# vmware/splinterdb

Hardware: AMD Instinct MI355X
Metric: routing_filter build Mkeys/s + probe Mkeys/s, device-resident, 24B keys (higher is better)
Workload: dtype u32; 1 GPU; C2: 64M x 24B keys per GPU = 8 filters x 8,000,000, build + full probe; filters_total=8, filters_per_gpu=8, keys_per_filter=8000000, key_len=24, fingerprint_size=26, log_index_size=8, seed=42, parallelism=key-range shards, 1 rank(s), no data-path collective

## Files before the change

### splinterdb_amd/csrc/rf_kernels.hip

```cpp
#include <hip/hip_runtime.h>
#include <stdint.h>

#include <atomic>

#include "rf_device.h"
#include "rf_plan.h"
#include "rf_launch.h"

using namespace rf;

typedef unsigned int v4u __attribute__((ext_vector_type(4)));
typedef unsigned int v2u __attribute__((ext_vector_type(2)));

template <int KIND, bool NT = false>
__device__ __forceinline__ uint32_t hash_key(const void* __restrict__ in0, const uint64_t* __restrict__ offs,
                                             uint32_t key_len, uint32_t seed, uint64_t k) {
  if constexpr (KIND == IN_KEYS24) {
    const v2u* kp = reinterpret_cast<const v2u*>(static_cast<const uint8_t*>(in0) + k * 24);
    v2u a, b, c;
    if constexpr (NT) {
      a = __builtin_nontemporal_load(kp);
      b = __builtin_nontemporal_load(kp + 1);
      c = __builtin_nontemporal_load(kp + 2);
    } else {
      a = kp[0];
      b = kp[1];
      c = kp[2];
    }
    uint32_t w[6] = {a.x, a.y, b.x, b.y, c.x, c.y};
    return xxh32_24(w, seed);
  } else if constexpr (KIND == IN_KEYS_W) {
    return xxh32_words(reinterpret_cast<const uint32_t*>(static_cast<const uint8_t*>(in0) + k * key_len),
                       key_len, seed);
  } else if constexpr (KIND == IN_KEYS_B) {
    const uint8_t* kp = static_cast<const uint8_t*>(in0) + k * key_len;
    return NT ? xxh32_unaligned_prefetch(kp, key_len, seed) : xxh32_unaligned(kp, key_len, seed);
  } else if constexpr (KIND == IN_VAR) {
    const uint64_t o0 = offs[k], o1 = offs[k + 1];
    const uint8_t* kp = static_cast<const uint8_t*>(in0) + o0;
    return NT ? xxh32_unaligned_prefetch(kp, (uint32_t)(o1 - o0), seed) : xxh32_unaligned(kp, (uint32_t)(o1 - o0), seed);
  } else {
    if constexpr (NT) return __builtin_nontemporal_load(static_cast<const uint32_t*>(in0) + k);
    else return static_cast<const uint32_t*>(in0)[k];
  }
}

#define KEY_KIND_CASES(L)              \
  case IN_KEYS24: L(IN_KEYS24); break; \
  case IN_KEYS_W: L(IN_KEYS_W); break; \
  case IN_KEYS_B: L(IN_KEYS_B); break; \
  case IN_VAR: L(IN_VAR); break;
#define KIND_SWITCH(kind, L)    \
  switch (kind) {               \
    KEY_KIND_CASES(L)           \
    default: L(IN_HASH); break; \
  }

__device__ __forceinline__ uint32_t select64_fast(uint64_t x, uint32_t r) {
  uint32_t pos = 0;
#pragma unroll
  for (uint32_t w = 32; w >= 1; w >>= 1) {
    const uint32_t c = __popcll(x & ((1ull << w) - 1));
    if (r >= c) { r -= c; x >>= w; pos += w; }
  }
  return pos;
}
__device__ __forceinline__ uint64_t lowmask64(uint32_t k) { return k >= 64 ? ~0ull : ((1ull << k) - 1); }

__device__ __forceinline__ uint32_t xcd_chunk(uint32_t b, uint32_t nb) {
  const uint32_t q = nb / 8, r = nb % 8, xcd = b % 8;
  return (xcd < r ? xcd * (q + 1) : r * (q + 1) + (xcd - r) * q) + b / 8;
}

__device__ __forceinline__ void cb_scan_filter(const FilterPlan& P, const uint32_t* counts, uint32_t* cb_count,
                                               uint32_t* cb_start, uint32_t* cb_cursor, uint32_t* s_tmp,
                                               bool fresh) {
  const uint32_t num_cb = 1u << P.cbits;
  constexpr uint32_t PER = MAX_CB / 256;
  uint32_t v[PER], sum = 0;
#pragma unroll
  for (uint32_t k = 0; k < PER; k++) {
    const uint32_t i = threadIdx.x * PER + k;
    v[k] = 0;
    if (i < num_cb)
      v[k] = fresh ? __hip_atomic_load(&counts[P.cb_base + i], __ATOMIC_RELAXED, __HIP_MEMORY_SCOPE_AGENT)
                   : counts[P.cb_base + i];
    sum += v[k];
  }
  uint32_t total;
  uint32_t run = block_excl_scan<256>(sum, s_tmp, &total);
#pragma unroll
  for (uint32_t k = 0; k < PER; k++) {
    const uint32_t i = threadIdx.x * PER + k;
    if (i < num_cb) {
      cb_count[P.cb_base + i] = v[k];
      cb_start[P.cb_base + i] = run;
      cb_cursor[P.cb_base + i] = run;
    }
    run += v[k];
  }
}

struct TileRuns {
  const uint32_t* value;
  const uint32_t* end;
};

struct CountFold {
  uint32_t* outs_words;
  uint32_t num_out_words;
  uint32_t* ticket;
  uint32_t* cb_count;
  uint32_t* cb_start;
  uint32_t num_filters;
};

template <int KIND, typename EntT, bool FL = (sizeof(EntT) == 8), bool RUNS = false>
__global__ __launch_bounds__(TILE_NT) void k_hash_count(const FilterPlan* __restrict__ plans,
                                                        const uint32_t* __restrict__ tile_filter,
                                                        const uint32_t* __restrict__ tile_start,
                                                        const void* __restrict__ in0,
                                                        const uint64_t* __restrict__ offs,
                                                        uint32_t key_len, uint32_t fp_size,
                                                        uint32_t seed, EntT* __restrict__ ent,
                                                        uint32_t* cb_count,
                                                        const uint32_t* __restrict__ gate, uint32_t num_tiles,
                                                        CountFold fold, TileRuns runs) {
  __shared__ uint32_t s_hist[MAX_CB];
  if (fold.outs_words && blockIdx.x == 0)
    for (uint32_t i = threadIdx.x; i < fold.num_out_words; i += TILE_NT) fold.outs_words[i] = 0;
  if (gate && *gate == 0) return;
  for (uint32_t t = blockIdx.x; t < num_tiles; t += gridDim.x) {
  const FilterPlan& P = plans[tile_filter[t]];
  const uint32_t start = tile_start[t];
  const uint32_t count = RUNS ? runs.end[t] - start : min((uint32_t)TILE_KEYS, P.num_new - start);
  const uint32_t value = RUNS ? runs.value[t] : P.value;
  const uint32_t num_cb = 1u << P.cbits;
  __syncthreads();
  for (uint32_t i = threadIdx.x; i < num_cb; i += TILE_NT) s_hist[i] = 0;
  __syncthreads();
  const uint32_t esh = fp_size + P.vs - P.cbits;
  for (uint32_t j = threadIdx.x; j < count; j += TILE_NT) {
    const uint32_t h = hash_key<KIND>(in0, offs, key_len, seed, P.key_first + start + j);
    const uint32_t e = ((h >> (32 - fp_size)) << P.vs) | value;
    if constexpr (FL) {
      ent[P.e_first + start + j] = (EntT)(((EntT)e << 1) | EntT(1));
    } else {
      ent[P.e_first + start + j] = e;
    }
    const uint32_t cb = P.cbits ? (e >> esh) : 0u;
    atomicAdd(&s_hist[cb], 1u);
  }
  __syncthreads();
  for (uint32_t i = threadIdx.x; i < num_cb; i += TILE_NT) {
    const uint32_t c = s_hist[i];
    if (c) atomicAdd(&cb_count[P.cb_base + i], c);
  }
  }
  if (fold.ticket) {
    static_assert(TILE_NT == 256, "cb_scan_filter's workgroup");
    __shared__ uint32_t s_last;
    __threadfence();
    __syncthreads();
    if (threadIdx.x == 0) s_last = atomicAdd(fold.ticket, 1u) == gridDim.x - 1 ? 1u : 0u;
    __syncthreads();
    if (!s_last) return;
    __threadfence();
    if (threadIdx.x == 0) *fold.ticket = 0;
    for (uint32_t f = 0; f < fold.num_filters; f++)
      cb_scan_filter(plans[f], cb_count, fold.cb_count, fold.cb_start, cb_count, s_hist, true);
  }
}

__global__ __launch_bounds__(TILE_NT) void k_old_count(const FilterPlan* __restrict__ plans,
                                                       const uint32_t* __restrict__ tile_filter,
                                                       const uint32_t* __restrict__ tile_start,
                                                       uint32_t fp_size,
                                                       const uint64_t* __restrict__ ent,
                                                       uint32_t* __restrict__ cb_count) {
  __shared__ uint32_t s_hist[MAX_CB];
  const uint32_t t = blockIdx.x;
  const FilterPlan& P = plans[tile_filter[t]];
  const uint32_t start = tile_start[t];
  const uint32_t count = min((uint32_t)TILE_KEYS, P.old_region - start);
  const uint32_t num_cb = 1u << P.cbits;
  for (uint32_t i = threadIdx.x; i < num_cb; i += TILE_NT) s_hist[i] = 0;
  __syncthreads();
  const uint32_t esh = fp_size + P.vs - P.cbits;
  for (uint32_t j = threadIdx.x; j < count; j += TILE_NT) {
    const uint64_t x = ent[P.e_first + P.num_new + start + j];
    if (x == ~0ull) continue;
    const uint32_t e = (uint32_t)(x >> 1);
    atomicAdd(&s_hist[P.cbits ? (e >> esh) : 0u], 1u);
  }
  __syncthreads();
  for (uint32_t i = threadIdx.x; i < num_cb; i += TILE_NT) {
    const uint32_t c = s_hist[i];
    if (c) atomicAdd(&cb_count[P.cb_base + i], c);
  }
}

__global__ __launch_bounds__(256) void k_cb_scan(const FilterPlan* __restrict__ plans,
                                                 const uint32_t* counts,
                                                 uint32_t* cb_count,
                                                 uint32_t* __restrict__ cb_start,
                                                 uint32_t* cb_cursor,
                                                 const uint32_t* __restrict__ gate) {
  __shared__ uint32_t s_tmp[256 / WAVE + 1];
  if (gate && *gate == 0) return;
  cb_scan_filter(plans[blockIdx.x], counts, cb_count, cb_start, cb_cursor, s_tmp, false);
}

template <typename EntT, bool FL = (sizeof(EntT) == 8), bool RUNS = false>
__global__ __launch_bounds__(SCAT_NT) void k_scatter(const FilterPlan* __restrict__ plans,
                                                     const uint32_t* __restrict__ tile_filter,
                                                     const uint32_t* __restrict__ tile_start,
                                                     uint32_t region_is_old, uint32_t fp_size,
                                                     const EntT* __restrict__ ent,
                                                     EntT* __restrict__ part,
                                                     uint32_t* __restrict__ cb_cursor,
                                                     const uint32_t* __restrict__ gate, uint32_t num_tiles,
                                                     TileRuns runs) {
  __shared__ EntT s_stage[TILE_KEYS];
  __shared__ uint32_t s_off[MAX_CB];
  __shared__ uint32_t s_tmp[SCAT_NT / WAVE + 1];
  if (gate && *gate == 0) return;
  constexpr int PER = TILE_KEYS / SCAT_NT;
  constexpr int BPT = MAX_CB / SCAT_NT;
  for (uint32_t t = blockIdx.x; t < num_tiles; t += gridDim.x) {
  __syncthreads();
  const FilterPlan& P = plans[tile_filter[t]];
  const uint32_t start = tile_start[t];
  const uint32_t region = region_is_old ? P.old_region : P.num_new;
  const uint64_t base = P.e_first + (region_is_old ? P.num_new : 0u) + start;
  const uint32_t count = (RUNS && !region_is_old) ? runs.end[t] - start : min((uint32_t)TILE_KEYS, region - start);
  const uint32_t num_cb = 1u << P.cbits;
  for (uint32_t i = threadIdx.x; i < num_cb; i += SCAT_NT) s_off[i] = 0;
  __syncthreads();
  const uint32_t esh = fp_size + P.vs - P.cbits;
  auto cb_of = [&](EntT x) -> uint32_t {
    uint32_t e;
    if constexpr (FL) e = (uint32_t)(x >> 1);
    else e = x;
    return P.cbits ? (e >> esh) : 0u;
  };
  EntT v[PER];
  uint32_t cbv[PER], rank[PER];
#pragma unroll
  for (int k = 0; k < PER; k++) v[k] = ent[base + min(threadIdx.x + k * SCAT_NT, count - 1)];
#pragma unroll
  for (int k = 0; k < PER; k++) {
    const uint32_t j = threadIdx.x + k * SCAT_NT;
    cbv[k] = ~0u;
    if (j < count) {
      bool valid = true;
      if constexpr (sizeof(EntT) == 8) valid = v[k] != ~0ull;
      if (valid) {
        cbv[k] = cb_of(v[k]);
        rank[k] = atomicAdd(&s_off[cbv[k]], 1u);
      }
    }
  }
  __syncthreads();
  uint32_t cnt[BPT], sum = 0;
#pragma unroll
  for (int k = 0; k < BPT; k++) {
    const uint32_t b = threadIdx.x * BPT + k;
    cnt[k] = b < num_cb ? s_off[b] : 0u;
    sum += cnt[k];
  }
  uint32_t valid_total;
  uint32_t run = block_excl_scan<SCAT_NT>(sum, s_tmp, &valid_total);
  uint32_t gbase[BPT];
#pragma unroll
  for (int k = 0; k < BPT; k++) {
    const uint32_t b = threadIdx.x * BPT + k;
    gbase[k] = 0;
    if (b < num_cb) {
      s_off[b] = run;
      if (cnt[k]) gbase[k] = atomicAdd(&cb_cursor[P.cb_base + b], cnt[k]) - run;
      run += cnt[k];
    }
  }
  __syncthreads();
#pragma unroll
  for (int k = 0; k < PER; k++) {
    if (cbv[k] != ~0u) s_stage[s_off[cbv[k]] + rank[k]] = v[k];
  }
  __syncthreads();
#pragma unroll
  for (int k = 0; k < BPT; k++) {
    const uint32_t b = threadIdx.x * BPT + k;
    if (b < num_cb) s_off[b] = gbase[k];
  }
  __syncthreads();
  EntT* dst = part + P.e_first;
  for (uint32_t j = threadIdx.x; j < valid_total; j += SCAT_NT) {
    const EntT x = s_stage[j];
    dst[s_off[cb_of(x)] + j] = x;
  }
  }
}

__device__ uint64_t* g_dbg_ts = nullptr;
__device__ uint32_t g_dbg_kid = 0;
#ifdef RF_PHASE_STAMPS
#define DBG_PHASE_K(kid, k)                                                  \
  do {                                                                       \
    uint64_t* _ts = g_dbg_ts;                                                \
    if (_ts && g_dbg_kid == (kid) && threadIdx.x == 0)                       \
      _ts[blockIdx.x * 16 + (k)] = __builtin_amdgcn_s_memtime();             \
  } while (0)
#else
#define DBG_PHASE_K(kid, k) \
  do {                      \
  } while (0)
#endif
#define DBG_PHASE(k) DBG_PHASE_K(1, k)

extern "C" int rf_debug_set_phase_buffer(uint64_t* d_buf, uint32_t kid) {
  if (hipMemcpyToSymbol(HIP_SYMBOL(g_dbg_kid), &kid, sizeof(kid)) != hipSuccess) return 1;
  return hipMemcpyToSymbol(HIP_SYMBOL(g_dbg_ts), &d_buf, sizeof(d_buf)) == hipSuccess ? 0 : 1;
}

#ifndef RF_SCAT_WPE
#define RF_SCAT_WPE 4
#endif
template <int KIND, bool FL = false, bool RUNS = false, bool P16 = false>
__global__ __launch_bounds__(SCAT_NT) __attribute__((amdgpu_waves_per_eu(RF_SCAT_WPE))) void k_hash_scatter(const FilterPlan* __restrict__ plans,
                                                          const uint32_t* __restrict__ tile_filter,
                                                          const uint32_t* __restrict__ tile_start,
                                                          const void* __restrict__ in0,
                                                          const uint64_t* __restrict__ offs,
                                                          uint32_t key_len, uint32_t fp_size, uint32_t seed,
                                                          uint32_t* __restrict__ part,
                                                          uint32_t* __restrict__ cb_fill,
                                                          uint32_t* __restrict__ spill, TileRuns runs) {
  __shared__ __attribute__((aligned(16))) uint32_t s_stage[TILE_KEYS];
  __shared__ uint32_t s_off[MAX_CB];
  __shared__ uint32_t s_tmp[SCAT_NT / WAVE + 1];
  constexpr int PER = TILE_KEYS / SCAT_NT;
  constexpr int BPT = MAX_CB / SCAT_NT;
  static_assert(!P16 || (!FL && !RUNS), "16-bit keys: fresh single-run builds only");
  DBG_PHASE_K(2, 15);
  const uint32_t t = xcd_chunk(blockIdx.x, gridDim.x);
  const FilterPlan& P = plans[tile_filter[t]];
  const uint32_t start = tile_start[t];
  const uint32_t count = RUNS ? runs.end[t] - start : min((uint32_t)TILE_KEYS, P.num_new - start);
  const uint32_t value = RUNS ? runs.value[t] : P.value;
  const uint32_t num_cb = 1u << P.cbits;
  for (uint32_t i = threadIdx.x; i < num_cb; i += SCAT_NT) s_off[i] = 0;
  __syncthreads();
  DBG_PHASE_K(2, 0);
  const uint32_t esh = fp_size + P.vs - P.cbits + (FL ? 1u : 0u);
  auto cb_of = [&](uint32_t e) -> uint32_t { return P.cbits ? (e >> esh) : 0u; };
  const uint32_t flag = FL ? 1u : 0u;
  uint32_t v[PER], rank[PER];
  constexpr int HASH_CHUNK = 8;
  uint32_t dep = 0;
  constexpr bool X3 = KIND == IN_KEYS24;
  const uint32_t lane = threadIdx.x & (WAVE - 1);
  auto key_of = [&](int k) -> uint32_t {
    if constexpr (KIND == IN_VAR) return (threadIdx.x & ~(WAVE - 1)) * PER + k * WAVE + lane;
    else if constexpr (X3) return (threadIdx.x & ~(WAVE - 1)) + k * SCAT_NT + (lane >> 1) + (lane & 1) * 32;
    else return threadIdx.x + k * SCAT_NT;
  };
  constexpr uint32_t VWIN = (TILE_KEYS / (SCAT_NT / WAVE)) * 4 - 16;
  uint32_t* s_vwin = s_stage + (threadIdx.x / WAVE) * (TILE_KEYS / (SCAT_NT / WAVE));
  uint64_t vw0 = 0, vw1 = 0, vo0 = 0, vo1 = 0;
  if constexpr (KIND == IN_VAR) {
    const uint32_t j = min(key_of(0), count - 1);
    vo0 = offs[P.key_first + start + j];
    vo1 = offs[P.key_first + start + j + 1];
  }
#pragma unroll
  for (int k0 = 0; k0 < PER; k0 += HASH_CHUNK) {
    if constexpr (X3) {
      const uint32_t half = lane & 1, ki = lane >> 1;
      const uint8_t* kbase = static_cast<const uint8_t*>(in0) + (uint64_t)(P.key_first + start) * 24 + 12 * half;
      uint32_t a[HASH_CHUNK][3], b[HASH_CHUNK][3];
#pragma unroll
      for (int k = 0; k < HASH_CHUNK; k++) {
        const uint32_t c0 = (threadIdx.x & ~(WAVE - 1)) + (k0 + k) * SCAT_NT;
        const uint32_t ja = min(c0 + ki, count - 1) + dep, jb = min(c0 + 32 + ki, count - 1) + dep;
        const uint32_t* pa = reinterpret_cast<const uint32_t*>(kbase + (uint64_t)ja * 24);
        const uint32_t* pb = reinterpret_cast<const uint32_t*>(kbase + (uint64_t)jb * 24);
        a[k][0] = pa[0]; a[k][1] = pa[1]; a[k][2] = pa[2];
        b[k][0] = pb[0]; b[k][1] = pb[1]; b[k][2] = pb[2];
      }
#pragma unroll
      for (int k = 0; k < HASH_CHUNK; k++) {
        uint32_t w[6];
#pragma unroll
        for (int q = 0; q < 3; q++) {
          const uint32_t send = half ? a[k][q] : b[k][q];
          const uint32_t recv = (uint32_t)__builtin_amdgcn_mov_dpp((int)send, 0xB1, 0xf, 0xf, false);
          w[q] = half ? recv : a[k][q];
          w[3 + q] = half ? b[k][q] : recv;
        }
        const uint32_t h = xxh32_24(w, seed);
        v[k0 + k] = ((((h >> (32 - fp_size)) << P.vs) | value) << flag) | flag;
      }
    } else if constexpr (KIND == IN_KEYS24) {
      v2u ka[HASH_CHUNK], kb[HASH_CHUNK], kc[HASH_CHUNK];
#pragma unroll
      for (int k = 0; k < HASH_CHUNK; k++) {
        const uint32_t j = min(threadIdx.x + (k0 + k) * SCAT_NT, count - 1) + dep;
        const v2u* kp = reinterpret_cast<const v2u*>(static_cast<const uint8_t*>(in0) +
                                                     (uint64_t)(P.key_first + start + j) * 24);
        ka[k] = kp[0];
        kb[k] = kp[1];
        kc[k] = kp[2];
      }
      uint32_t z;
      asm volatile("v_mov_b32 %0, 0" : "=v"(z)
                   : "v"(ka[0].x), "v"(ka[1].x), "v"(ka[2].x), "v"(ka[3].x), "v"(ka[4].x), "v"(ka[5].x),
                     "v"(ka[6].x), "v"(ka[7].x), "v"(kb[0].x), "v"(kb[1].x), "v"(kb[2].x), "v"(kb[3].x),
                     "v"(kb[4].x), "v"(kb[5].x), "v"(kb[6].x), "v"(kb[7].x), "v"(kc[0].x), "v"(kc[1].x),
                     "v"(kc[2].x), "v"(kc[3].x), "v"(kc[4].x), "v"(kc[5].x), "v"(kc[6].x), "v"(kc[7].x));
#pragma unroll
      for (int k = 0; k < HASH_CHUNK; k++) {
        uint32_t w[6] = {ka[k].x + z, ka[k].y, kb[k].x, kb[k].y, kc[k].x, kc[k].y};
        const uint32_t h = xxh32_24(w, seed);
        v[k0 + k] = ((((h >> (32 - fp_size)) << P.vs) | value) << flag) | flag;
      }
    } else if constexpr (KIND == IN_VAR) {
#pragma unroll
      for (int k = 0; k < HASH_CHUNK; k++) {
        const uint64_t o0 = vo0, o1 = vo1;
        if (k0 + k + 1 < PER) {
          const uint32_t j = min(key_of(k0 + k + 1), count - 1);
          vo0 = offs[P.key_first + start + j];
          vo1 = offs[P.key_first + start + j + 1];
        }
        const uint32_t h = wave_hash_var<VWIN, false>(static_cast<const uint8_t*>(in0), o0, o1,
                                                      key_of(k0 + k) < count, s_vwin, seed, &vw0, &vw1);
        v[k0 + k] = ((((h >> (32 - fp_size)) << P.vs) | value) << flag) | flag;
      }
    } else {
#pragma unroll
      for (int k = k0; k < k0 + HASH_CHUNK; k++) {
        const uint32_t j = min(threadIdx.x + k * SCAT_NT, count - 1) + dep;
        const uint32_t h = hash_key<KIND>(in0, offs, key_len, seed, P.key_first + start + j);
        v[k] = ((((h >> (32 - fp_size)) << P.vs) | value) << flag) | flag;
      }
    }
    static_assert(HASH_CHUNK == 8, "opaque dependency below takes 8 hashes");
    asm volatile("v_mov_b32 %0, 0" : "=v"(dep)
                 : "v"(v[k0]), "v"(v[k0 + 1]), "v"(v[k0 + 2]), "v"(v[k0 + 3]), "v"(v[k0 + 4]),
                   "v"(v[k0 + 5]), "v"(v[k0 + 6]), "v"(v[k0 + 7]));
  }
  DBG_PHASE_K(2, 5);
#pragma unroll
  for (int k = 0; k < PER; k++) {
    if (key_of(k) < count) rank[k] = atomicAdd(&s_off[cb_of(v[k])], 1u);
  }
  __syncthreads();
  DBG_PHASE_K(2, 1);
  uint32_t cnt[BPT], sum = 0;
#pragma unroll
  for (int k = 0; k < BPT; k++) {
    const uint32_t b = threadIdx.x * BPT + k;
    cnt[k] = b < num_cb ? s_off[b] : 0u;
    sum += cnt[k];
  }
  uint32_t total;
  uint32_t run = block_excl_scan<SCAT_NT>(sum, s_tmp, &total);
  uint32_t g[BPT], lstart[BPT];
#pragma unroll
  for (int k = 0; k < BPT; k++) {
    const uint32_t b = threadIdx.x * BPT + k;
    g[k] = 0;
    lstart[k] = run;
    if (b < num_cb) {
      if (cnt[k]) g[k] = atomicAdd(&cb_fill[P.cb_base + b], cnt[k]);
      s_off[b] = run;
      run += cnt[k];
    }
  }
  __syncthreads();
  DBG_PHASE_K(2, 2);
#pragma unroll
  for (int k = 0; k < PER; k++) {
    if (key_of(k) < count) s_stage[s_off[cb_of(v[k])] + rank[k]] = v[k];
  }
  __syncthreads();
  DBG_PHASE_K(2, 3);
  bool over = false;
#pragma unroll
  for (int k = 0; k < BPT; k++) {
    const uint32_t b = threadIdx.x * BPT + k;
    if (b < num_cb) {
      over |= cnt[k] && g[k] + cnt[k] > (uint32_t)SORT_CAP;
      s_off[b] = g[k] - lstart[k];
    }
  }
  if (over) atomicOr(spill, 1u);
  __syncthreads();
  DBG_PHASE_K(2, 4);
  uint32_t* dst = part + P.e_first;
  if constexpr (P16) {
    auto reg16 = [&](uint32_t cb) -> uint16_t* { return reinterpret_cast<uint16_t*>(dst + (uint64_t)cb * CB_REGION); };
    for (uint32_t j = threadIdx.x; j < total; j += SCAT_NT) {
      const uint32_t x = s_stage[j];
      const uint32_t cb = cb_of(x);
      const uint32_t slot = s_off[cb] + j;
      if (slot < (uint32_t)SORT_CAP) reg16(cb)[slot] = (uint16_t)x;
    }
  } else {
    for (uint32_t j = threadIdx.x; j < total; j += SCAT_NT) {
      const uint32_t x = s_stage[j];
      const uint32_t cb = cb_of(x);
      const uint32_t slot = s_off[cb] + j;
      if (slot < (uint32_t)SORT_CAP) dst[(uint64_t)cb * CB_REGION + slot] = x;
    }
  }
  DBG_PHASE_K(2, 8);
}

template <typename EntT, bool FL = (sizeof(EntT) == 8)>
__device__ __forceinline__ uint32_t ent_e(EntT x) {
  if constexpr (FL) return (uint32_t)(x >> 1);
  else return x;
}
template <typename EntT, bool FL = (sizeof(EntT) == 8)>
__device__ __forceinline__ bool ent_drop(EntT x, EntT prev) {
  if constexpr (FL) return x == prev && (x & EntT(1));
  else return x == prev;
}

template <typename T>
__device__ __forceinline__ void sort8(T (&x)[8]) {
#define CE(a, b) { const T lo = x[a] < x[b] ? x[a] : x[b], hi = x[a] < x[b] ? x[b] : x[a]; x[a] = lo; x[b] = hi; }
  CE(0, 1) CE(2, 3) CE(4, 5) CE(6, 7) CE(0, 2) CE(1, 3) CE(4, 6) CE(5, 7) CE(1, 2) CE(5, 6)
  CE(0, 4) CE(1, 5) CE(2, 6) CE(3, 7) CE(2, 4) CE(3, 5) CE(1, 2) CE(3, 4) CE(5, 6)
#undef CE
}
template <typename T>
__device__ __forceinline__ void sort16(T (&x)[16]) {
#define CE(a, b) { const T lo = x[a] < x[b] ? x[a] : x[b], hi = x[a] < x[b] ? x[b] : x[a]; x[a] = lo; x[b] = hi; }
  CE(0, 1) CE(2, 3) CE(0, 2) CE(1, 3) CE(1, 2) CE(4, 5) CE(6, 7) CE(4, 6) CE(5, 7) CE(5, 6) CE(0, 4)
  CE(2, 6) CE(2, 4) CE(1, 5) CE(3, 7) CE(3, 5) CE(1, 2) CE(3, 4) CE(5, 6) CE(8, 9) CE(10, 11) CE(8, 10)
  CE(9, 11) CE(9, 10) CE(12, 13) CE(14, 15) CE(12, 14) CE(13, 15) CE(13, 14) CE(8, 12) CE(10, 14)
  CE(10, 12) CE(9, 13) CE(11, 15) CE(11, 13) CE(9, 10) CE(11, 12) CE(13, 14) CE(0, 8) CE(4, 12)
  CE(4, 8) CE(2, 10) CE(6, 14) CE(6, 10) CE(2, 4) CE(6, 8) CE(10, 12) CE(1, 9) CE(5, 13) CE(5, 9)
  CE(3, 11) CE(7, 15) CE(7, 11) CE(3, 5) CE(7, 9) CE(11, 13) CE(1, 2) CE(3, 4) CE(5, 6) CE(7, 8)
  CE(9, 10) CE(11, 12) CE(13, 14)
#undef CE
}

template <typename T, int NT>
__device__ void oe_sort_group(T* a, uint32_t cnt) {
  uint32_t n = 1;
  while (n < cnt) n <<= 1;
  for (uint32_t p = 1; p < n; p <<= 1) {
    for (uint32_t k = p; k >= 1; k >>= 1) {
      const uint32_t r = k & (p - 1);
      for (uint32_t L = threadIdx.x; L + k < cnt; L += NT) {
        if (L >= r && ((L - r) & (2 * k - 1)) < k && (L / (2 * p)) == ((L + k) / (2 * p))) {
          const T x = a[L], y = a[L + k];
          if (y < x) {
            a[L] = y;
            a[L + k] = x;
          }
        }
      }
      __syncthreads();
    }
  }
}

struct CbCtx {
  uint32_t rvs, vs, lis, bbits, idx0;
  uint32_t cb_rel;
  uint64_t e_first;
};

__device__ __forceinline__ void write_index_bounds(const CbCtx& c, const uint32_t* sorted, uint32_t kept,
                                                   uint32_t* idx_cnt, uint32_t* idx_start,
                                                   uint32_t* uniq_out) {
  const uint32_t ipc = 1u << (c.bbits - c.lis);
  const uint32_t ish = c.lis + c.rvs;
  for (uint32_t li = threadIdx.x; li < ipc; li += blockDim.x) {
    auto lb = [&](uint32_t key) {
      uint32_t lo = 0, hi = kept;
      while (lo < hi) {
        uint32_t mid = (lo + hi) >> 1;
        uint32_t m = ish >= 32 ? 0u : ((sorted[mid] >> ish) & (ipc - 1));
        if (m < key) lo = mid + 1; else hi = mid;
      }
      return lo;
    };
    const uint32_t lo = lb(li);
    const uint32_t hi = (li + 1 < ipc) ? lb(li + 1) : kept;
    idx_cnt[c.idx0 + li] = hi - lo;
    idx_start[c.idx0 + li] = c.cb_rel + lo;
  }
  uint32_t uniq = 0;
  for (uint32_t i = threadIdx.x; i < kept; i += blockDim.x) {
    const uint32_t fp = sorted[i] >> c.vs;
    const bool first = (i == 0) || (ish < 32 && ((sorted[i] >> ish) != (sorted[i - 1] >> ish)));
    const uint32_t prev = first ? (0xffffffffu >> c.vs) : (sorted[i - 1] >> c.vs);
    uniq += (fp != prev) ? 1u : 0u;
  }
  *uniq_out = uniq;
}

template <typename EntT, bool FL = (sizeof(EntT) == 8), bool DUAL = false, bool LIST = false, bool RUNS = false>
__global__ __launch_bounds__(SORT_NT, 6) void k_cb_sort(const FilterPlan* __restrict__ plans,
                                                     const uint32_t* __restrict__ cb_filter,
                                                     const uint32_t* __restrict__ cb_count,
                                                     const uint32_t* __restrict__ cb_start,
                                                     const EntT* __restrict__ part,
                                                     const uint32_t* __restrict__ old32,
                                                     const uint32_t* __restrict__ ob_lo,
                                                     const uint32_t* __restrict__ ob_n,
                                                     uint32_t* __restrict__ sorted32,
                                                     uint32_t* __restrict__ idx_cnt,
                                                     uint32_t* __restrict__ idx_start,
                                                     FilterOut* __restrict__ outs,
                                                     uint32_t* __restrict__ overflow,
                                                     uint32_t lis, uint32_t* __restrict__ first_old,
                                                     uint32_t* __restrict__ has_old,
                                                     const uint32_t* __restrict__ spill,
                                                     const uint32_t* __restrict__ cb_outs,
                                                     const uint32_t* __restrict__ cb_list) {
  constexpr int PER = SORT_CAP / SORT_NT;
  DBG_PHASE(15);
  __shared__ EntT s_b[SORT_CAP];
  __shared__ __attribute__((aligned(16))) uint32_t s_bin[MAX_BINS + 1];
  __shared__ uint32_t s_tmp[SORT_NT / WAVE + 1];
  static_assert(MAX_BINS + 1 >= 2048 + 2 * MAX_IPC && MAX_IPC + 1 <= 2048, "s_fo / s_ho inside s_bin");
  constexpr uint32_t BIG_LIST = 64;
  __shared__ uint32_t s_big[BIG_LIST];
  __shared__ uint32_t s_nbig;
  uint32_t* s_first = s_bin;
  uint32_t* s_fo = s_bin + 2048;
  uint32_t* s_ho = s_bin + 2048 + MAX_IPC;
  const uint32_t nit = LIST ? cb_list[0] : 1u;
  for (uint32_t it = LIST ? blockIdx.x : 0u; it < nit; it += LIST ? gridDim.x : 1u) {
  uint32_t cb;
  if constexpr (LIST) {
    cb = cb_list[1 + it];
    if (!(cb >> 31)) continue;
    cb &= 0x7fffffffu;
  } else {
    cb = xcd_chunk(blockIdx.x, gridDim.x);
  }
  const uint32_t f = cb_filter[cb];
  const FilterPlan& P = plans[f];
  const uint32_t n = cb_count[cb];
  const uint32_t cbl = cb - P.cb_base;
  const uint32_t cb_rel = (spill && *spill == 0) ? cbl * CB_REGION : cb_start[cb];
  const uint32_t cb_out = (DUAL && spill) ? cb_outs[cb] : cb_rel;
  CbCtx c{P.rvs, P.vs, lis, P.bbits, P.idx_base + (cbl << (P.bbits - lis)), cb_out, P.e_first};
  if (n > SORT_CAP) {
    if (threadIdx.x == 0 && !LIST) overflow[1 + atomicAdd(&overflow[0], 1u)] = cb;
    continue;
  }
  const uint32_t nbins = 1u << (P.bbits - P.binsh);
  const uint32_t bmask = nbins - 1, bsh = P.rvs + P.binsh;
  const uint32_t ipc = 1u << (P.bbits - lis), ish = lis + P.rvs;
  EntT v[PER];
  static_assert(SORT_CAP <= 65536 && PER % 2 == 0, "16-bit ranks, packed in pairs");
  uint32_t rp[PER / 2];
#pragma unroll
  for (int k = 0; k < PER / 2; k++) rp[k] = 0;
  const EntT* src = part + P.e_first + cb_rel;
  const uint32_t nm1 = n ? n - 1 : 0u;
  if constexpr (DUAL) {
    const uint32_t nn = n - ob_n[cb];
    const uint32_t* osrc = (P.old_direct ? P.old_entries : old32 + P.old_first) + ob_lo[cb];
#pragma unroll
    for (int k = 0; k < PER; k++) {
      const uint32_t j = min(threadIdx.x + k * SORT_NT, nm1);
      v[k] = *(j < nn ? reinterpret_cast<const uint32_t*>(src) + j : osrc + (j - nn));
    }
  } else {
#pragma unroll
    for (int k = 0; k < PER; k++) v[k] = src[min(threadIdx.x + k * SORT_NT, nm1)];
  }
  for (uint32_t i = threadIdx.x; i <= nbins; i += SORT_NT) s_bin[i] = 0;
  if (threadIdx.x == 0) s_nbig = 0;
  __builtin_amdgcn_fence(__ATOMIC_RELEASE, "workgroup", "local");
  __builtin_amdgcn_s_barrier();
  __builtin_amdgcn_fence(__ATOMIC_ACQUIRE, "workgroup", "local");
  DBG_PHASE(0);
  uint32_t nsort = n;
  if constexpr (DUAL) nsort = n - ob_n[cb];
#pragma unroll
  for (int k = 0; k < PER; k++) {
    if (threadIdx.x + k * SORT_NT < nsort) {
      const uint32_t e = ent_e<EntT, FL>(v[k]);
      const uint32_t b = bsh >= 32 ? 0u : ((e >> bsh) & bmask);
      rp[k / 2] |= atomicAdd(&s_bin[b], 1u) << (16 * (k & 1));
    }
  }
  __syncthreads();
  DBG_PHASE(1);
  {
    constexpr int BPT = MAX_BINS / SORT_NT;
    static_assert(BPT == 8, "two 16-byte accesses per thread");
    v4u* sb4 = reinterpret_cast<v4u*>(s_bin) + 2 * threadIdx.x;
    const bool own = threadIdx.x * BPT < nbins;
    v4u a = own ? sb4[0] : v4u{0u, 0u, 0u, 0u}, b = own ? sb4[1] : v4u{0u, 0u, 0u, 0u};
    if (own && nbins < BPT) {
      uint32_t t8[8] = {a.x, a.y, a.z, a.w, b.x, b.y, b.z, b.w};
#pragma unroll
      for (int k = 0; k < 8; k++) if ((uint32_t)k >= nbins) t8[k] = 0;
      a = v4u{t8[0], t8[1], t8[2], t8[3]};
      b = v4u{t8[4], t8[5], t8[6], t8[7]};
    }
    const uint32_t sum = a.x + a.y + a.z + a.w + b.x + b.y + b.z + b.w;
    uint32_t total;
    uint32_t run = block_excl_scan<SORT_NT>(sum, s_tmp, &total);
    v4u ea, eb;
    ea.x = run; run += a.x; ea.y = run; run += a.y; ea.z = run; run += a.z; ea.w = run; run += a.w;
    eb.x = run; run += b.x; eb.y = run; run += b.y; eb.z = run; run += b.z; eb.w = run;
    if (own && nbins >= BPT) {
      sb4[0] = ea;
      sb4[1] = eb;
    } else if (own) {
      const uint32_t e8[8] = {ea.x, ea.y, ea.z, ea.w, eb.x, eb.y, eb.z, eb.w};
      for (uint32_t k = 0; k < nbins; k++) s_bin[k] = e8[k];
    }
    if (threadIdx.x == 0) s_bin[nbins] = nsort;
  }
  __syncthreads();
  DBG_PHASE(2);
#pragma unroll
  for (int k = 0; k < PER; k++) {
    const uint32_t i = threadIdx.x + k * SORT_NT;
    if (i < nsort) {
      const uint32_t e = ent_e<EntT, FL>(v[k]);
      const uint32_t b = bsh >= 32 ? 0u : ((e >> bsh) & bmask);
      s_b[s_bin[b] + ((rp[k / 2] >> (16 * (k & 1))) & 0xffffu)] = v[k];
    } else if (i < n) {
      const uint32_t eo = (uint32_t)v[k];
      const uint32_t e = P.old_direct ? ((eo >> P.old_vs) << P.vs) | (eo & ((1u << P.old_vs) - 1u)) : eo;
      s_b[i] = (EntT)e << 1;
    }
  }
  __syncthreads();
  DBG_PHASE(3);
  {
    constexpr EntT EMAX = ~EntT(0);
    uint32_t S = 8;
    while (S > 1 && (uint64_t)S * nsort > 8ull * nbins) S >>= 1;
    if (S > nbins) S = nbins;
    const uint32_t nseg = nbins / S;
    for (uint32_t sg = threadIdx.x; sg < nseg; sg += SORT_NT) {
      const uint32_t b0 = sg * S, st = s_bin[b0], c = s_bin[b0 + S] - st;
      if (c <= 16) {
        EntT x[16];
#pragma unroll
        for (int j = 0; j < 16; j++) x[j] = (uint32_t)j < c ? s_b[st + j] : EMAX;
        sort16(x);
        if (c >= 2) {
// ... 4087 lines not shown
```

Measured before the change: 48630 Mkeys/s.

## Pipeline 24B key loads through an LDS DMA ring in hash-scatter

For full, 16-byte-aligned tiles of 24-byte keys, the hash-scatter kernel now streams keys through a 5-slot LDS ring filled by asynchronous global-to-LDS DMA. Each step hashes one slot, refills it, and fuses the shared-memory atomic rank increment with the next slot's reads in hand-written asm using explicit vmcnt/lgkmcnt waits. The aim is to overlap global key fetch with hashing and atomics, replacing batched register loads. This relies on precise wait counts and an LDS slice size, and partial or misaligned tiles still use the old path. keys24_issue_dma is only forward-declared here.

```diff
diff --git a/splinterdb_amd/csrc/rf_kernels.hip b/splinterdb_amd/csrc/rf_kernels.hip
--- a/splinterdb_amd/csrc/rf_kernels.hip
+++ b/splinterdb_amd/csrc/rf_kernels.hip
@@ -326,6 +326,19 @@
 #ifndef RF_SCAT_WPE
 #define RF_SCAT_WPE 4
 #endif
+__device__ __forceinline__ void keys24_issue_dma(const uint8_t* kb, v4u* sw, uint32_t lane);
+template <int VM>
+__device__ __forceinline__ void ring_read(uint64_t& x, uint64_t& y, uint64_t& z, uint32_t key) {
+  asm volatile("s_waitcnt vmcnt(%4)\n\tds_read_b64 %0, %3\n\tds_read_b64 %1, %3 offset:8\n\tds_read_b64 %2, %3 offset:16\n\t"
+               "s_waitcnt lgkmcnt(0)"
+               : "=&v"(x), "=&v"(y), "=&v"(z) : "v"(key), "n"(VM) : "memory");
+}
+template <int VM>
+__device__ __forceinline__ void ring_step(uint32_t& rank, uint64_t& x, uint64_t& y, uint64_t& z, uint32_t cnt, uint32_t key) {
+  asm volatile("ds_add_rtn_u32 %3, %5, %6\n\ts_waitcnt vmcnt(%7)\n\tds_read_b64 %0, %4\n\tds_read_b64 %1, %4 offset:8\n\t"
+               "ds_read_b64 %2, %4 offset:16\n\ts_waitcnt lgkmcnt(0)"
+               : "=&v"(x), "=&v"(y), "=&v"(z), "=&v"(rank) : "v"(key), "v"(cnt), "v"(1u), "n"(VM) : "memory");
+}
 template <int KIND, bool FL = false, bool RUNS = false, bool P16 = false>
 __global__ __launch_bounds__(SCAT_NT) __attribute__((amdgpu_waves_per_eu(RF_SCAT_WPE))) void k_hash_scatter(const FilterPlan* __restrict__ plans,
                                                           const uint32_t* __restrict__ tile_filter,
@@ -373,6 +386,48 @@
     vo0 = offs[P.key_first + start + j];
     vo1 = offs[P.key_first + start + j + 1];
   }
+  auto entry_of = [&](uint32_t h) -> uint32_t { return ((((h >> (32 - fp_size)) << P.vs) | value) << flag) | flag; };
+  bool piped = false;
+  if constexpr (X3) {
+    constexpr int RING = 5;
+    static_assert(RING == 5 && PER >= RING && RING * 96 * 16 <= (TILE_KEYS / (SCAT_NT / WAVE)) * 4, "waits below; slice size");
+    const uint8_t* tb = static_cast<const uint8_t*>(in0) + (uint64_t)(P.key_first + start) * 24;
+    piped = count == (uint32_t)TILE_KEYS && ((uintptr_t)tb & 15) == 0;
+    if (piped) {
+      v4u* sw = reinterpret_cast<v4u*>(s_vwin);
+      const uint8_t* kb = tb + (threadIdx.x & ~(WAVE - 1)) * 24;
+#pragma unroll
+      for (int r = 0; r < RING; r++) keys24_issue_dma(kb + r * (SCAT_NT * 24), sw + r * 96, lane);
+      const uint32_t lds_key = (uint32_t)(uintptr_t)(__attribute__((address_space(3))) uint8_t*)reinterpret_cast<uint8_t*>(sw) + lane * 24;
+      const uint32_t lds_off = (uint32_t)(uintptr_t)(__attribute__((address_space(3))) uint32_t*)s_off;
+      uint64_t x, y, z;
+      auto key_at = [&](int k) -> uint32_t { return lds_key + (k % RING) * 1536; };
+      auto hash_slot = [&](int k) {
+        wave_sync_lds();
+        if (k + RING < PER) keys24_issue_dma(kb + (k + RING) * (SCAT_NT * 24), sw + (k % RING) * 96, lane);
+        const uint32_t w[6] = {(uint32_t)x, (uint32_t)(x >> 32), (uint32_t)y, (uint32_t)(y >> 32), (uint32_t)z, (uint32_t)(z >> 32)};
+        v[k] = entry_of(xxh32_24(w, seed));
+        return lds_off + cb_of(v[k]) * 4;
+      };
+      ring_read<8>(x, y, z, key_at(0));
+#pragma unroll
+      for (int k = 0; k < PER - RING; k++) {
+        const uint32_t ao = hash_slot(k);
+        ring_step<8>(rank[k], x, y, z, ao, key_at(k + 1));
+      }
+      uint32_t ao = hash_slot(PER - 5);
+      ring_step<6>(rank[PER - 5], x, y, z, ao, key_at(PER - 4));
+      ao = hash_slot(PER - 4);
+      ring_step<4>(rank[PER - 4], x, y, z, ao, key_at(PER - 3));
+      ao = hash_slot(PER - 3);
+      ring_step<2>(rank[PER - 3], x, y, z, ao, key_at(PER - 2));
+      ao = hash_slot(PER - 2);
+      ring_step<0>(rank[PER - 2], x, y, z, ao, key_at(PER - 1));
+      ao = hash_slot(PER - 1);
+      asm volatile("ds_add_rtn_u32 %0, %1, %2\n\ts_waitcnt lgkmcnt(0)" : "=&v"(rank[PER - 1]) : "v"(ao), "v"(1u) : "memory");
+    }
+  }
+  if (!piped) {
 #pragma unroll
   for (int k0 = 0; k0 < PER; k0 += HASH_CHUNK) {
     if constexpr (X3) {
@@ -450,10 +505,13 @@
                  : "v"(v[k0]), "v"(v[k0 + 1]), "v"(v[k0 + 2]), "v"(v[k0 + 3]), "v"(v[k0 + 4]),
                    "v"(v[k0 + 5]), "v"(v[k0 + 6]), "v"(v[k0 + 7]));
   }
+  }
   DBG_PHASE_K(2, 5);
-#pragma unroll
-  for (int k = 0; k < PER; k++) {
-    if (key_of(k) < count) rank[k] = atomicAdd(&s_off[cb_of(v[k])], 1u);
+  if (!piped) {
+#pragma unroll
+    for (int k = 0; k < PER; k++) {
+      if (key_of(k) < count) rank[k] = atomicAdd(&s_off[cb_of(v[k])], 1u);
+    }
   }
   __syncthreads();
   DBG_PHASE_K(2, 1);
```

Measured after the change: 50110 Mkeys/s (median of 6 runs). 3.0% higher.
